# sieste/greb-climate-model

Measured on AMD Instinct MI355X. Metric: simulated-years/sec at 96x48 grid (ensemble aggregate); diffusion HBM GB/s vs roofline, higher is better.
Workload: dtype f32; 1 GPU; 96x48 GREB ensemble, 512 members/GPU x 1 GPU, CO2 sweep 280-1120 ppm, 32 scenario years after 1 flux-correction year, dt=12h, dt_crcl=0.5h; members_per_gpu=512, arithmetic=fast, gather=none (1 GPU)

## Files before the change

greb_climate_model_amd/csrc/greb_member.hip:

```cpp
#include <cstdlib>

#include "greb_kernels.h"
#include "greb_pair.h"
#include "greb_physics_step.h"
#include "greb_stencil.h"

namespace greb {

constexpr int NX = 96, NY = 48, NQ = 24, NP = 4608;
constexpr int kThreads = 512;
constexpr int RS = 2 * NX + 16;
constexpr int XB = (NY + 2) * RS;
constexpr int kOffX = RS;
constexpr int kOffW = 2 * XB + RS;
constexpr int kOffWX = 3 * XB;
constexpr int kOffWY = kOffWX + NP;
constexpr int kOffRowK = kOffWY + NP;
constexpr int kRowKCsDif = 7;
constexpr int kLdsFloats = kOffRowK + NY * kRowKWords;
constexpr size_t kLdsBytes = (size_t)kLdsFloats * sizeof(float);

bool member_layout_supported(const RowTables& t, int nx, int ny) {
  if (nx != NX || ny != NY) return false;
  for (int k = 0; k < NY; ++k) {
    const bool sub = (k <= 9 || k >= 38);
    if ((t.subcycled[k] != 0) != sub) return false;
    const bool chain = (k == 0 || k == NY - 1);
    if ((t.dif_time2[k] > 1 || t.adv_time2[k] > 1) != chain) return false;
  }
  if (t.dif_time2[0] != t.dif_time2[NY - 1] || t.adv_time2[0] != t.adv_time2[NY - 1]) return false;
  return true;
}

__device__ __forceinline__ f4 comp(const q8& q, int tr) {
  return tr == 0 ? f4{{q.v[0].x, q.v[1].x, q.v[2].x, q.v[3].x}} : f4{{q.v[0].y, q.v[1].y, q.v[2].y, q.v[3].y}};
}
__device__ __forceinline__ q8 zip(const f4& a, const f4& b) {
  q8 r;
#pragma unroll
  for (int i = 0; i < 4; ++i) r.v[i] = v2{a.v[i], b.v[i]};
  return r;
}

struct TaskAddr { int c, l, r, kq; };

__device__ __forceinline__ q8 ld8p(const lfloat* p) {
  const vfloat4 a = *(const __attribute__((address_space(3))) vfloat4*)p;
  const vfloat4 b = *(const __attribute__((address_space(3))) vfloat4*)(p + kHalfRow);
  q8 r;
  r.v[0] = v2{a.x, a.y}; r.v[1] = v2{a.z, a.w}; r.v[2] = v2{b.x, b.y}; r.v[3] = v2{b.z, b.w};
  return r;
}

template <bool SUB>
__device__ __forceinline__ q8 fast_row(const q8& LT, const q8& CT, const q8& RT, const q8& Tm2, const q8& Tm1, const q8& Tp1,
                                       const q8& Tp2, const q8& LW, const q8& CW, const q8& RW, const q8& Wm2, const q8& Wm1,
                                       const q8& Wp1, const q8& Wp2, const f4& xq, const f4& yq, const WindSigns& ws,
                                       bool last_quad, float cs_dif, float dif_ccy, bool calm_q) {
  v2 T[12], w[12];
#pragma unroll
  for (int j = 0; j < 4; ++j) {
    T[j] = LT.v[j]; T[4 + j] = CT.v[j]; T[8 + j] = RT.v[j];
    w[j] = LW.v[j]; w[4 + j] = CW.v[j]; w[8 + j] = RW.v[j];
  }
  return substep_pair<SUB>(T, w, Tm2, Tm1, Tp1, Tp2, Wm2, Wm1, Wp1, Wp2, xq.v, ws.x, yq.v, ws.y, cs_dif, dif_ccy, last_quad, calm_q);
}

__device__ __forceinline__ void st8p(lfloat* o, const q8& xn) {
  vfloat4 a, b;
  a.x = xn.v[0].x; a.y = xn.v[0].y; a.z = xn.v[1].x; a.w = xn.v[1].y;
  b.x = xn.v[2].x; b.y = xn.v[2].y; b.z = xn.v[3].x; b.w = xn.v[3].y;
  *(__attribute__((address_space(3))) vfloat4*)o = a;
  *(__attribute__((address_space(3))) vfloat4*)(o + kHalfRow) = b;
}

__device__ __forceinline__ q8 strict_row(const q8& LT, const q8& CT, const q8& RT, const q8& Tm2, const q8& Tm1, const q8& Tp1,
                                         const q8& Tp2, const q8& LW, const q8& CW, const q8& RW, const q8& Wm2, const q8& Wm1,
                                         const q8& Wp1, const q8& Wp2, const f4& xq, const f4& yq, int k, int q,
                                         const RowK& rk, bool calm_q) {
#pragma clang fp contract(off)
  q8 xn;
  v2 T[12], w[12];
#pragma unroll
  for (int j = 0; j < 4; ++j) {
    T[j] = LT.v[j]; T[4 + j] = CT.v[j]; T[8 + j] = RT.v[j];
    w[j] = LW.v[j]; w[4 + j] = CW.v[j]; w[8 + j] = RW.v[j];
  }
  v2 dTx[4], dTy[4], dd[4], da[4];
  dif_lon_strict(T, w, rk.dif_cc, dTx);
  if (rk.sub) {
    v2 T1h[4] = {T[4], T[5], T[6], T[7]};
    clamp_add(T1h, dTx);
#pragma unroll
    for (int i = 0; i < 4; ++i) dTx[i] = T1h[i] - T[4 + i];
  }
  dif_lat_strict(CT, Tm1, Tp1, Wm1, Wp1, rk.dif_ccy, k, NY, dTy);
#pragma unroll
  for (int i = 0; i < 4; ++i) dd[i] = CW.v[i] * (dTx[i] + dTy[i]);
  if (!rk.sub) {
    adv_lon_full_strict(T, w, xq.v, rk.adv_cc, dTx);
  } else {
    v2 T1h[4] = {T[4], T[5], T[6], T[7]};
    adv_lon_sub_strict(T, w, xq.v, rk.adv_cc, q == NQ - 1, dTx);
    clamp_add(T1h, dTx);
#pragma unroll
    for (int i = 0; i < 4; ++i) dTx[i] = T1h[i] - T[4 + i];
  }
  adv_lat_strict(CT, Tm2, Tm1, Tp1, Tp2, Wm2, Wm1, Wp1, Wp2, yq.v, rk.adv_ccy, k, NY, dTy);
#pragma unroll
  for (int i = 0; i < 4; ++i) {
    da[i] = dTx[i] + dTy[i];
    const v2 xd = T[4 + i] + dd[i];
    v2 x = xd + da[i];
    if (calm_q) x.y = xd.y;
    xn.v[i] = x;
  }
  return xn;
}

template <bool STRICT, bool SUB>
__device__ __forceinline__ q8 one_row(const q8& LT, const q8& CT, const q8& RT, const q8& Tm2, const q8& Tm1, const q8& Tp1,
                                      const q8& Tp2, const q8& LW, const q8& CW, const q8& RW, const q8& Wm2, const q8& Wm1,
                                      const q8& Wp1, const q8& Wp2, const f4& xq, const f4& yq, const WindSigns& ws, int k, int q,
                                      const RowK& rk, bool calm_q) {
  if (STRICT) return strict_row(LT, CT, RT, Tm2, Tm1, Tp1, Tp2, LW, CW, RW, Wm2, Wm1, Wp1, Wp2, xq, yq, k, q, rk, calm_q);
  return fast_row<SUB>(LT, CT, RT, Tm2, Tm1, Tp1, Tp2, LW, CW, RW, Wm2, Wm1, Wp1, Wp2, xq, yq, ws, q == NQ - 1, rk.dif_cc,
                       rk.dif_ccy, calm_q);
}

template <bool STRICT>
__device__ __forceinline__ RowK task_consts(const lfloat* lds, int k, float ccy_dif) {
  if (STRICT) return row_consts((const lfloat*)(lds + kOffRowK), k);
  RowK rk{};
  rk.dif_cc = lds[kOffRowK + k * kRowKWords + kRowKCsDif];
  rk.dif_ccy = ccy_dif;
  return rk;
}

template <bool STRICT, bool SUB>
__device__ __forceinline__ void row_task(lfloat* lds, int cur, const TaskAddr& ta, const WindSigns* ws, float ccy_dif,
                                         bool calm_q = false) {
  const int k = ta.kq & 255, q = ta.kq >> 8;
  const lfloat* Xc = lds + kOffX + cur * XB;
  const lfloat* Wc = lds + kOffW;
  const RowK rk = task_consts<STRICT>(lds, k, ccy_dif);
  const f4 xq = ld4(lds + kOffWX + k * NX + 4 * q), yq = ld4(lds + kOffWY + k * NX + 4 * q);
  const lfloat* xb = Xc + ta.c - 2 * RS;
  const lfloat* wb = Wc + ta.c - 2 * RS;
  const q8 Tm2 = ld8p(xb), Tm1 = ld8p(xb + RS), CT = ld8p(xb + 2 * RS), Tp1 = ld8p(xb + 3 * RS), Tp2 = ld8p(xb + 4 * RS);
  const q8 Wm2 = ld8p(wb), Wm1 = ld8p(wb + RS), CW = ld8p(wb + 2 * RS), Wp1 = ld8p(wb + 3 * RS), Wp2 = ld8p(wb + 4 * RS);
  const q8 LT = ld8p(Xc + ta.l), RT = ld8p(Xc + ta.r), LW = ld8p(Wc + ta.l), RW = ld8p(Wc + ta.r);
  const q8 xn = one_row<STRICT, SUB>(LT, CT, RT, Tm2, Tm1, Tp1, Tp2, LW, CW, RW, Wm2, Wm1, Wp1, Wp2, xq, yq, ws[0], k, q, rk,
                                     calm_q);
  st8p(lds + kOffX + (cur ^ 1) * XB + ta.c, xn);
}

template <bool STRICT, bool SUB>
__device__ __forceinline__ void row_task2(lfloat* lds, int cur, const TaskAddr& ta, const WindSigns* ws, float ccy_dif,
                                          bool calm_q = false) {
  const int k = ta.kq & 255, q = ta.kq >> 8;
  const lfloat* Xc = lds + kOffX + cur * XB;
  const lfloat* Wc = lds + kOffW;
  const lfloat* xb = Xc + ta.c - 2 * RS;
  const lfloat* wb = Wc + ta.c - 2 * RS;
  const q8 T0 = ld8p(xb), T1 = ld8p(xb + RS), T2 = ld8p(xb + 2 * RS), T3 = ld8p(xb + 3 * RS), T4 = ld8p(xb + 4 * RS);
  const q8 W0 = ld8p(wb), W1 = ld8p(wb + RS), W2 = ld8p(wb + 2 * RS), W3 = ld8p(wb + 3 * RS), W4 = ld8p(wb + 4 * RS);
  lfloat* out = lds + kOffX + (cur ^ 1) * XB + ta.c;
  {
    const q8 LT = ld8p(Xc + ta.l), RT = ld8p(Xc + ta.r), LW = ld8p(Wc + ta.l), RW = ld8p(Wc + ta.r);
    const f4 xq = ld4(lds + kOffWX + k * NX + 4 * q), yq = ld4(lds + kOffWY + k * NX + 4 * q);
    const RowK rk = task_consts<STRICT>(lds, k, ccy_dif);
    st8p(out, one_row<STRICT, SUB>(LT, T2, RT, T0, T1, T3, T4, LW, W2, RW, W0, W1, W3, W4, xq, yq, ws[0], k, q, rk, calm_q));
  }
  __builtin_amdgcn_sched_barrier(0);
  {
    const q8 T5 = ld8p(xb + 5 * RS), W5 = ld8p(wb + 5 * RS);
    const q8 LT = ld8p(Xc + ta.l + RS), RT = ld8p(Xc + ta.r + RS), LW = ld8p(Wc + ta.l + RS), RW = ld8p(Wc + ta.r + RS);
    const f4 xq = ld4(lds + kOffWX + (k + 1) * NX + 4 * q), yq = ld4(lds + kOffWY + (k + 1) * NX + 4 * q);
    const RowK rk = task_consts<STRICT>(lds, k + 1, ccy_dif);
    st8p(out + RS,
         one_row<STRICT, SUB>(LT, T3, RT, T1, T2, T4, T5, LW, W3, RW, W1, W2, W4, W5, xq, yq, ws[1], k + 1, q, rk, calm_q));
  }
}

struct BulkTasks { TaskAddr t[3]; };
struct BulkSigns { WindSigns s[3][2]; };

enum { kNone = 0, kS1 = 1, kF1 = 2, kST = 3, kFT = 4 };
struct Pass { int kind, index; };
__host__ __device__ constexpr Pass deal_fast(int wave, int i) {
  constexpr Pass none{kNone, 0};
#if defined(GREB_TUNING) && defined(GREB_DEAL_FAST)
  constexpr Pass t[8][3] = {GREB_DEAL_FAST};
#else
  constexpr Pass t[8][3] = {
       {{kST, 0}, {kF1, 0}, none},      {{kST, 2}, {kF1, 1}, none},
       {{kFT, 1}, {kF1, 3}, none},      {{kFT, 2}, {kS1, 0}, none},
       {{kST, 1}, none, none},          {{kFT, 0}, none, none},
       {none, none, none},              {{kF1, 2}, {kF1, 4}, none}};
#endif
  return t[wave][i];
}
__host__ __device__ constexpr Pass deal_strict(int wave, int i) {
  constexpr Pass none{kNone, 0};
  constexpr Pass t[8][3] = {
       {{kST, 0}, {kFT, 0}, none},      {{kST, 2}, {kF1, 0}, {kF1, 1}},
       {none, none, none},              {none, none, none},
       {{kST, 1}, none, none},          {{kF1, 2}, {kF1, 3}, none},
       {{kFT, 1}, {kS1, 0}, none},      {{kFT, 2}, {kF1, 4}, none}};
  return t[wave][i];
}
template <bool STRICT>
__host__ __device__ constexpr Pass deal(int wave, int i) { return STRICT ? deal_strict(wave, i) : deal_fast(wave, i); }
#if defined(GREB_TUNING) && defined(GREB_POLAR_WAVE_FAST)
constexpr int kPolarWaveFast = GREB_POLAR_WAVE_FAST;
#else
constexpr int kPolarWaveFast = 6;
#endif
template <bool STRICT>
__host__ __device__ constexpr bool is_polar_wave(int wave) { return STRICT ? (wave == 2 || wave == 3) : wave == kPolarWaveFast; }

struct RowQuad { int k, q, valid; };
__host__ __device__ constexpr int task_rows(int kind) { return kind == kST || kind == kFT ? 2 : (kind == kS1 || kind == kF1 ? 1 : 0); }
__host__ __device__ constexpr RowQuad task_rowquad(int kind, int t) {
  int k = 1, q = 0, valid = 0;
  const int r = t / NQ;
  q = t % NQ;
  if (kind == kST) { valid = r < 8; k = r < 4 ? 1 + 2 * r : (r == 4 ? 41 : (r == 5 ? 39 : (r == 6 ? 45 : 43))); }
  else if (kind == kFT) { valid = r < 8; k = 10 + 2 * r; }
  else if (kind == kS1) { valid = r < 2; k = r == 0 ? 9 : 38; if (r == 1) q = (q + 4) % NQ; }
  else if (kind == kF1) { valid = r < 12; k = r < 6 ? 26 + 2 * r : 27 + 2 * (r - 6); }
  if (!valid) { k = 1; q = 0; }
  return RowQuad{k, q, valid};
}

__host__ __device__ constexpr int kind_passes(int kind) { return kind == kST || kind == kFT ? 3 : (kind == kS1 ? 1 : (kind == kF1 ? 5 : 0)); }
__host__ __device__ constexpr int pass_tasks(int kind, int index) {
  const int total = kind == kST || kind == kFT ? 8 * NQ : (kind == kS1 ? 2 * NQ : (kind == kF1 ? 12 * NQ : 0));
  const int left = total - 64 * index;
  return left >= 64 ? 64 : (left > 0 ? left : 0);
}

struct DealCover { int n[NY * NQ]; };
template <bool STRICT>
__host__ __device__ constexpr DealCover deal_cover() {
  DealCover c{};
  for (int w = 0; w < 8; ++w)
    for (int i = 0; i < 3; ++i) {
      const Pass p = deal<STRICT>(w, i);
      if (p.kind == kNone) continue;
      for (int lane = 0; lane < 64; ++lane) {
        const RowQuad rq = task_rowquad(p.kind, 64 * p.index + lane);
        for (int j = 0; j < (rq.valid ? task_rows(p.kind) : 0); ++j) ++c.n[(rq.k + j) * NQ + rq.q];
      }
    }
  return c;
}
template <bool STRICT>
__host__ __device__ constexpr bool deal_is_complete() {
  for (int w = 0; w < 8; ++w)
    for (int i = 0; i < 3; ++i) {
      const Pass p = deal<STRICT>(w, i);
      if (is_polar_wave<STRICT>(w) && p.kind != kNone) return false;
      if (p.kind != kNone && (p.index < 0 || p.index >= kind_passes(p.kind))) return false;
    }
  const DealCover c = deal_cover<STRICT>();
  for (int k = 0; k < NY; ++k)
    for (int q = 0; q < NQ; ++q) if (c.n[k * NQ + q] != (k >= 1 && k <= NY - 2 ? 1 : 0)) return false;
  return true;
}
static_assert(deal_is_complete<true>() && deal_is_complete<false>(),
              "a deal must compute every row-quad of rows 1 .. 46 exactly once and give the polar waves no bulk pass");

void member_deal_cover(bool strict, int* counts) {
  constexpr DealCover cs = deal_cover<true>(), cf = deal_cover<false>();
  for (int i = 0; i < NY * NQ; ++i) counts[i] = strict ? cs.n[i] : cf.n[i];
}

template <bool STRICT>
__device__ __forceinline__ BulkTasks make_tasks(int wave, int lane) {
  BulkTasks b;
#pragma unroll
  for (int i = 0; i < 3; ++i) {
    const RowQuad rq = task_rowquad(deal<STRICT>(wave, i).kind, deal<STRICT>(wave, i).index * 64 + lane);
    const int k = rq.k, q = rq.q, valid = rq.valid;
    TaskAddr a;
    a.c = k * RS + 4 * q;
    a.l = k * RS + 4 * (q == 0 ? NQ - 1 : q - 1);
    a.r = k * RS + 4 * (q == NQ - 1 ? 0 : q + 1);
    a.kq = valid ? (k | (q << 8)) : -1;
    asm volatile("" : "+v"(a.c), "+v"(a.l), "+v"(a.r), "+v"(a.kq));
    b.t[i] = a;
  }
  return b;
}

template <int WAVE>
__device__ __forceinline__ void make_signs(const lfloat* lds, const BulkTasks& tasks, BulkSigns& b) {
  static_for<3>([&](auto I) {
    constexpr int i = I, rows = task_rows(deal_fast(WAVE, i).kind);
    if constexpr (rows > 0) {
      const int kq = tasks.t[i].kq < 0 ? 1 : tasks.t[i].kq, k = kq & 255, q = kq >> 8;
#pragma unroll
      for (int j = 0; j < rows; ++j) {
        const f4 xq = ld4(lds + kOffWX + (k + j) * NX + 4 * q), yq = ld4(lds + kOffWY + (k + j) * NX + 4 * q);
#pragma unroll
        for (int e = 0; e < 4; ++e) {
          unsigned long long mx = __builtin_amdgcn_ballot_w64(xq.v[e] > 0.f), my = __builtin_amdgcn_ballot_w64(yq.v[e] > 0.f);
          asm volatile("" : "+s"(mx), "+s"(my));
          b.s[i][j].x[e] = mx; b.s[i][j].y[e] = my;
        }
      }
    }
  });
}

template <bool STRICT, int SLOT, int I>
__device__ __forceinline__ void bulk_task(lfloat* lds, int cur, const BulkTasks& tasks, const BulkSigns& signs, float ccy_dif,
                                          int dbg, bool calm_q) {
  constexpr int kind = deal<STRICT>(SLOT, I).kind, ntask = pass_tasks(kind, deal<STRICT>(SLOT, I).index);
  if constexpr (kind != kNone && ntask > 0) {
    if (ntask < 64 && tasks.t[I].kq < 0) return;
    if constexpr (kind == kS1) { if (!(dbg & 1)) row_task<STRICT, true>(lds, cur, tasks.t[I], signs.s[I], ccy_dif, calm_q); }
    else if constexpr (kind == kF1) { if (!(dbg & 2)) row_task<STRICT, false>(lds, cur, tasks.t[I], signs.s[I], ccy_dif, calm_q); }
    else if constexpr (kind == kST) { if (!(dbg & 1)) row_task2<STRICT, true>(lds, cur, tasks.t[I], signs.s[I], ccy_dif, calm_q); }
    else { if (!(dbg & 2)) row_task2<STRICT, false>(lds, cur, tasks.t[I], signs.s[I], ccy_dif, calm_q); }
  }
}
template <bool STRICT, int SLOT>
__device__ __forceinline__ void bulk_substep(lfloat* lds, int cur, const BulkTasks& tasks, const BulkSigns& signs, float ccy_dif,
                                             int dbg, bool calm_q = false) {
  bulk_task<STRICT, SLOT, 0>(lds, cur, tasks, signs, ccy_dif, dbg, calm_q);
  bulk_task<STRICT, SLOT, 1>(lds, cur, tasks, signs, ccy_dif, dbg, calm_q);
  bulk_task<STRICT, SLOT, 2>(lds, cur, tasks, signs, ccy_dif, dbg, calm_q);
}

__device__ __forceinline__ int pair_off(int l) { return (l & 1) * kHalfRow + (l >> 1) * 4; }
__device__ __forceinline__ void load_win10(const lfloat* row, int l, v2 t[10]) {
  const int lm2 = l >= 2 ? l - 2 : l + 46, lm1 = l >= 1 ? l - 1 : 47, lp1 = l <= 46 ? l + 1 : 0, lp2 = l <= 45 ? l + 2 : l - 46;
  const int idx[5] = {lm2, lm1, l, lp1, lp2};
#pragma unroll
  for (int i = 0; i < 5; ++i) {
    const vfloat4 a = *(const __attribute__((address_space(3))) vfloat4*)(row + pair_off(idx[i]));
    t[2 * i] = v2{a.x, a.y}; t[2 * i + 1] = v2{a.z, a.w};
  }
}
__device__ __forceinline__ void st_pair2(lfloat* p, v2 a, v2 b) {
  vfloat4 x; x.x = a.x; x.y = a.y; x.z = b.x; x.w = b.y;
  *(__attribute__((address_space(3))) vfloat4*)p = x;
}

__device__ __forceinline__ void chain_substep_strict(lfloat* lds, int cur, int pole, int l , bool calm_q = false) {
  if (l >= 48) return;
  const int k = pole ? NY - 1 : 0;
  const RowK rk = row_consts((const lfloat*)(lds + kOffRowK), k);
  const lfloat* Xc = lds + kOffX + cur * XB;
  const lfloat* Wc = lds + kOffW;
  v2 T0w[10], w[10];
  load_win10(Xc + k * RS, l, T0w);
  load_win10(Wc + k * RS, l, w);
  const float u0 = lds[kOffWX + k * NX + 2 * l], u1 = lds[kOffWX + k * NX + 2 * l + 1];
  const float v0 = lds[kOffWY + k * NX + 2 * l], v1 = lds[kOffWY + k * NX + 2 * l + 1];
  const int k1 = pole ? k - 1 : k + 1, k2 = pole ? k - 2 : k + 2;
  v2 T1[2], T2[2], W1[2], W2[2];
  {
    const vfloat4 a = *(const __attribute__((address_space(3))) vfloat4*)(Xc + k1 * RS + pair_off(l));
    const vfloat4 b = *(const __attribute__((address_space(3))) vfloat4*)(Xc + k2 * RS + pair_off(l));
    const vfloat4 c = *(const __attribute__((address_space(3))) vfloat4*)(Wc + k1 * RS + pair_off(l));
    const vfloat4 d = *(const __attribute__((address_space(3))) vfloat4*)(Wc + k2 * RS + pair_off(l));
    T1[0] = v2{a.x, a.y}; T1[1] = v2{a.z, a.w}; T2[0] = v2{b.x, b.y}; T2[1] = v2{b.z, b.w};
    W1[0] = v2{c.x, c.y}; W1[1] = v2{c.z, c.w}; W2[0] = v2{d.x, d.y}; W2[1] = v2{d.z, d.w};
  }
  const v2 own[2] = {T0w[4], T0w[5]};
  const bool bug_lane = (l == 46);
  const int am2 = 4 * (l >= 2 ? l - 2 : l + 46), am1 = 4 * (l >= 1 ? l - 1 : 47), ap1 = 4 * (l <= 46 ? l + 1 : 0),
            ap2 = 4 * (l <= 45 ? l + 2 : l - 46);
  auto from = [](int addr, v2 x) {
    return v2{__int_as_float(__builtin_amdgcn_ds_bpermute(addr, __float_as_int(x.x))),
              __int_as_float(__builtin_amdgcn_ds_bpermute(addr, __float_as_int(x.y)))};
  };
  const float uu[2] = {u0, u1};

  v2 Th[2][2];
#pragma unroll
  for (int which = 0; which < 2; ++which) {
    const int time2 = __builtin_amdgcn_readfirstlane(which ? rk.adv_time2 : rk.dif_time2);
    const float cc = which ? rk.adv_cc : rk.dif_cc;
    v2 T[10];
#pragma unroll
    for (int i = 0; i < 10; ++i) T[i] = T0w[i];
    v2 th[2] = {own[0], own[1]};
    for (int tt = 0; tt < time2; ++tt) {
      if (tt > 0) {
        T[1] = from(am2, th[1]); T[2] = from(am1, th[0]); T[3] = from(am1, th[1]);
        T[4] = th[0]; T[5] = th[1];
        T[6] = from(ap1, th[0]); T[7] = from(ap1, th[1]); T[8] = from(ap2, th[0]);
      }
#pragma unroll
      for (int pt = 0; pt < 2; ++pt) {
#pragma clang fp contract(off)
        const int c = 4 + pt;
        v2 dd;
        if (which) dd = adv_lon_sub_point_strict(T, w, uu[pt], cc, c, bug_lane && pt == 1);
        else dd = div20(cc * dif_S_strict(T, w, c));
        dd = clamp_e(dd, T[c]);
        th[pt] = T[c] + dd;
      }
    }
    Th[which][0] = th[0]; Th[which][1] = th[1];
  }

  v2 xn[2];
  const float vv[2] = {v0, v1};
#pragma unroll
  for (int pt = 0; pt < 2; ++pt) {
#pragma clang fp contract(off)
    const v2 t0 = own[pt], w0 = w[4 + pt], a1 = T1[pt], a2 = T2[pt], b1 = W1[pt], b2 = W2[pt];
    const float vm = split_m(vv[pt]), vp = split_p(vv[pt]);
    v2 dTy, aTy;
    if (pole == 0) {
      dTy = rk.dif_ccy * b1 * (-t0 + a1);
      aTy = div3(rk.adv_ccy * (vp * (b1 * (t0 - a1) + b2 * (t0 - a2))));
    } else {
      dTy = rk.dif_ccy * b1 * (a1 - t0);
      aTy = div3(rk.adv_ccy * (-vm * (b1 * (t0 - a1) + b2 * (t0 - a2))));
    }
    const v2 dd = w0 * ((Th[0][pt] - t0) + dTy);
    const v2 da = (Th[1][pt] - t0) + aTy;
    const v2 xd = t0 + dd;
    v2 x = xd + da;
    if (calm_q) x.y = xd.y;
    xn[pt] = x;
  }
  st_pair2(lds + kOffX + (cur ^ 1) * XB + k * RS + pair_off(l), xn[0], xn[1]);
}

struct QuadChain {
  ChainK kd, ka;
  float w0[6], W1[6], W2[6];
  float own[6];
  float cv[6];
  float ccy;
  int at[3];
  int row[3];
  int time2_dif, time2_adv;
  bool calm;
};

__device__ __forceinline__ void quad_chain_setup(const lfloat* lds, int cur, int lane, bool calm_q, QuadChain& c) {
  const int r = lane >> 4, j = lane & 15, pole = r >> 1, C = r & 1;
  const int k = pole ? NY - 1 : 0, k1 = pole ? k - 1 : k + 1, k2 = pole ? k - 2 : k + 2;
  const RowK rk = row_consts((const lfloat*)(lds + kOffRowK), k);
  c.time2_dif = rk.dif_time2; c.time2_adv = rk.adv_time2; c.ccy = rk.dif_ccy;
  c.calm = calm_q && C == 1;
  c.row[0] = k * RS; c.row[1] = k1 * RS; c.row[2] = k2 * RS;
#pragma unroll
  for (int t = 0; t < 3; ++t) c.at[t] = pair_off(3 * j + t) + C;
  const lfloat* Wc = lds + kOffW;
  float w[12];
  static_for<12>([&](auto I) {
    constexpr int i = I;
    int x = 6 * j - 3 + i;
    x = x < 0 ? x + NX : (x >= NX ? x - NX : x);
    w[i] = Wc[c.row[0] + pair_off(x >> 1) + (x & 1) * 2 + C];
  });
  const float third = rk.adv_ccy * (1.f / 3.f), csd = rk.dif_cc * 0.05f, csa = rk.adv_cc * 0.05f;
  float Kd[6][6], Ka[6][6];
  static_for<6>([&](auto I) {
    constexpr int i = I, p = 3 + i;
    const int o = c.at[i >> 1] + (i & 1) * 2;
    c.w0[i] = w[p];
    c.own[i] = lds[kOffX + cur * XB + c.row[0] + o];
    c.W1[i] = Wc[c.row[1] + o];
    c.W2[i] = Wc[c.row[2] + o];
    const float u = lds[kOffWX + k * NX + 6 * j + i], v = lds[kOffWY + k * NX + 6 * j + i];
    c.cv[i] = pole == 0 ? third * fminf(v, 0.f) : -third * fmaxf(v, 0.f);
    Kd[i][0] = -csd * w[p - 3]; Kd[i][1] = (-3.f * csd) * w[p - 2]; Kd[i][2] = (-6.f * csd) * w[p - 1];
    Kd[i][3] = (6.f * csd) * w[p + 1]; Kd[i][4] = (3.f * csd) * w[p + 2]; Kd[i][5] = csd * w[p + 3];
    const float um = csa * fmaxf(u, 0.f), up = csa * fminf(u, 0.f);
    Ka[i][0] = -um * w[p - 3]; Ka[i][1] = (-4.f * um) * w[p - 2]; Ka[i][2] = (-10.f * um) * w[p - 1];
    Ka[i][3] = (-10.f * up) * w[p + 1]; Ka[i][4] = (-4.f * up) * w[p + 2]; Ka[i][5] = -up * w[p + 3];
    if (i == 3 && j == 15) {
      Ka[i][4] = -up * w[p + 3]; Ka[i][5] = -up * w[p + 3];
    }
  });
  c.kd = chain_pack(Kd);
  c.ka = chain_pack(Ka);
}

__device__ __forceinline__ void quad_chain_substep(lfloat* lds, int cur, QuadChain& c) {
  const lfloat* Xc = lds + kOffX + cur * XB;
  float own[6], T1[6], T2[6];
#pragma unroll
  for (int i = 0; i < 6; ++i) {
    const int o = c.at[i >> 1] + (i & 1) * 2;
    own[i] = c.own[i];
    T1[i] = Xc[c.row[1] + o];
    T2[i] = Xc[c.row[2] + o];
  }
  float Td[6], Ta[6];
#pragma unroll
  for (int i = 0; i < 6; ++i) { Td[i] = own[i]; Ta[i] = own[i]; }
  chain_run6<true>(Td, c.kd, c.time2_dif);
  chain_run6<true>(Ta, c.ka, c.time2_adv);
  lfloat* out = lds + kOffX + (cur ^ 1) * XB + c.row[0];
#pragma unroll
  for (int i = 0; i < 6; ++i) {
    const float g1 = c.W1[i] * (T1[i] - own[i]);
    const float d2 = c.W2[i] * (own[i] - T2[i]);
    const float ddy = c.ccy * g1;
    const float day = c.cv[i] * (d2 - g1);
    const float dd = c.w0[i] * ((Td[i] - own[i]) + ddy);
    float da = (Ta[i] - own[i]) + day;
    if (c.calm) da = 0.f;
    c.own[i] = (own[i] + dd) + da;
    out[c.at[i >> 1] + (i & 1) * 2] = c.own[i];
  }
}

template <bool STRICT, bool REMAT = false>
__device__ __forceinline__ void stage_winds(lfloat* lds, const float* __restrict__ u, const float* __restrict__ v,
                                            const RowTables* __restrict__ tab) {
  int tid0 = threadIdx.x;
  if (REMAT) asm volatile("" : "+v"(tid0));
  constexpr int kIt = (NP / 4 + kThreads - 1) / kThreads;
  f4 uq[kIt], vq[kIt];
#pragma unroll
  for (int j = 0; j < kIt; ++j) {
    const int i = min(tid0 + j * kThreads, NP / 4 - 1);
    uq[j] = ld4(u + 4 * i); vq[j] = ld4(v + 4 * i);
  }
#pragma unroll
  for (int j = 0; j < kIt; ++j) {
    const int i = tid0 + j * kThreads;
    if (i < NP / 4) {
      const int k = i / NQ;
      if (!(STRICT || k == 0 || k == NY - 1)) {
        const RowK rk = row_consts((const lfloat*)(lds + kOffRowK), k);
        const float cu = rk.sub ? rk.adv_cc * 0.05f : rk.adv_cc * (1.f / 3.f);
        const float cv = rk.adv_ccy * (1.f / 3.f);
#pragma unroll
        for (int e = 0; e < 4; ++e) { uq[j].v[e] *= cu; vq[j].v[e] *= cv; }
        if (k == 1 || k == NY - 2) {
#pragma unroll
          for (int e = 0; e < 4; ++e) {
            const float y = vq[j].v[e];
            vq[j].v[e] = (k == 1 ? y > 0.f : y < 0.f) ? 3.f * y : y;
          }
        }
      }
      st4(lds + kOffWX + 4 * i, uq[j]); st4(lds + kOffWY + 4 * i, vq[j]);
    }
  }
  (void)tab;
}

template <bool STRICT>
struct Circ {
  __device__ __forceinline__ void init(lfloat* lds, const float* wz_air, const float* wz_vapor,
                                       const RowTables* __restrict__ tab) {
    for (int i = threadIdx.x; i < 6 * RS; i += kThreads) {
      const int g = i / RS, o = i % RS;
      lds[(g >> 1) * XB + (g & 1) * (NY + 1) * RS + o] = 0.f;
    }
    stage_row_consts(lds + kOffRowK, *tab, 0, NY);
    if (!STRICT)
      for (int k = threadIdx.x; k < NY; k += blockDim.x)
        lds[kOffRowK + k * kRowKWords + kRowKCsDif] = lds[kOffRowK + k * kRowKWords] * 0.05f;
    for (int i = threadIdx.x; i < NP / 4; i += kThreads)
      st8(lds + kOffW + (i / NQ) * RS, i % NQ, zip(ld4(wz_air + 4 * i), ld4(wz_vapor + 4 * i)));
  }

  template <int WAVE, bool NOT_CALM>
  __device__ __forceinline__ void role_loop(lfloat* lds, int cur, int nsub, int lane, int dbg, bool calm_runtime
#ifdef GREB_TUNING
                                            , bool stamp, unsigned long long& busy
#endif
  ) {
    const bool calm_q = NOT_CALM ? false : calm_runtime;
    constexpr bool kPolar = is_polar_wave<STRICT>(WAVE);
    BulkTasks tasks;
    BulkSigns signs;
    QuadChain quad;
    if constexpr (!kPolar) tasks = make_tasks<STRICT>(WAVE, lane);
    else if constexpr (!STRICT) quad_chain_setup(lds, cur, lane, calm_q, quad);
    if constexpr (!kPolar && !STRICT) make_signs<WAVE>(lds, tasks, signs);
    float ccy_dif = 0.f;
    if constexpr (!kPolar && !STRICT) ccy_dif = __int_as_float(__builtin_amdgcn_readfirstlane(__float_as_int(lds[kOffRowK + 2])));
#pragma unroll 1
    for (int tt = 0; tt < nsub; ++tt) {
#ifdef GREB_TUNING
      const unsigned long long t0 = stamp ? __builtin_amdgcn_s_memtime() : 0;
#endif
      if constexpr (kPolar && STRICT) { if (!(dbg & 4)) chain_substep_strict(lds, cur, WAVE - 2, lane, calm_q); }
      else if constexpr (kPolar) { if (!(dbg & 4)) quad_chain_substep(lds, cur, quad); }
      else bulk_substep<STRICT, WAVE>(lds, cur, tasks, signs, ccy_dif, dbg, calm_q);
#ifdef GREB_TUNING
      if (stamp) busy += __builtin_amdgcn_s_memtime() - t0;
#endif
      __syncthreads();
      cur ^= 1;
    }
  }
  __device__ __forceinline__ void substeps(lfloat* lds, int cur, int nsub, int dbg = 0, bool calm_q = false
#ifdef GREB_TUNING
                                           , bool stamp = false, unsigned long long* busy = nullptr
#endif
  ) {
    int lane = threadIdx.x & 63;
    asm volatile("" : "+v"(lane));
#ifdef GREB_TUNING
    unsigned long long b = 0;
#define GREB_ROLE(W) case W: if (!STRICT && !calm_q) role_loop<W, true>(lds, cur, nsub, lane, dbg, false, stamp, b); \
                             else role_loop<W, false>(lds, cur, nsub, lane, dbg, calm_q, stamp, b); break;
#else
#define GREB_ROLE(W) case W: if (!STRICT && !calm_q) role_loop<W, true>(lds, cur, nsub, lane, dbg, false); \
                             else role_loop<W, false>(lds, cur, nsub, lane, dbg, calm_q); break;
#endif
    switch (__builtin_amdgcn_readfirstlane(threadIdx.x >> 6)) {
      GREB_ROLE(0) GREB_ROLE(1) GREB_ROLE(2) GREB_ROLE(3) GREB_ROLE(4) GREB_ROLE(5) GREB_ROLE(6) GREB_ROLE(7)
    }
#undef GREB_ROLE
#ifdef GREB_TUNING
    if (busy) *busy += b;
#endif
  }
};

template <bool STRICT>
__global__ __launch_bounds__(kThreads) void circulation_g96_kernel(const float* __restrict__ Xin,
                                                                   const float* __restrict__ wz,
                                                                   const float* __restrict__ ug,
                                                                   const float* __restrict__ vg,
                                                                   float* __restrict__ dX,
                                                                   const RowTables* __restrict__ tab, int nsub,
                                                                   int dbg) {
  extern __shared__ __align__(16) float lds_raw[];
  lfloat* lds = (lfloat*)lds_raw;
  const size_t fo = (size_t)blockIdx.x * NP;
  Circ<STRICT> c;
  c.init(lds, wz + fo, wz + fo, tab);
  for (int i = threadIdx.x; i < NP / 4; i += kThreads) {
    const f4 x = ld4(Xin + fo + 4 * i);
    st8(lds + kOffX + (i / NQ) * RS, i % NQ, zip(x, x));
  }
  __syncthreads();
  stage_winds<STRICT>(lds, ug + fo, vg + fo, tab);
  __syncthreads();
  c.substeps(lds, 0, nsub, dbg);
  const int cur = nsub & 1;
  for (int i = threadIdx.x; i < NP / 4; i += kThreads) {
    const f4 a = comp(ld8(lds + kOffX + cur * XB + (i / NQ) * RS, i % NQ), 0), b = ld4(Xin + fo + 4 * i);
    st4(dX + fo + 4 * i, f4{{a.v[0] - b.v[0], a.v[1] - b.v[1], a.v[2] - b.v[2], a.v[3] - b.v[3]}});
  }
}

hipError_t launch_circulation_g96(const float* X, const float* wz, const float* u, const float* v, float* dX,
                                  const RowTables* tab_dev, int batch, int nsub, bool strict, hipStream_t s) {
  auto kern = strict ? circulation_g96_kernel<true> : circulation_g96_kernel<false>;
  hipError_t e = hipFuncSetAttribute(reinterpret_cast<const void*>(kern),
                                     hipFuncAttributeMaxDynamicSharedMemorySize, (int)kLdsBytes);
  if (e != hipSuccess) return e;
  hipLaunchKernelGGL(kern, dim3(batch), dim3(kThreads), kLdsBytes, s, X, wz, u, v, dX, tab_dev, nsub,
                     tuning_int("GREB_DEBUG_SKIP", 0));
  return hipGetLastError();
}

template <bool STRICT, unsigned V>
__global__ __launch_bounds__(kThreads) void member_kernel(MemberArgs a) {
  constexpr bool FLUX = V & kVFlux, EXP = V & kVExp, BUDGET = V & kVBudget, FORCE = V & kVForce, BOUND = V & kVBound;
  extern __shared__ __align__(16) float lds_raw[];
  lfloat* lds = (lfloat*)lds_raw;
  const int m = blockIdx.x, tid = threadIdx.x;
  float* state = a.state + (size_t)m * 5 * NP;
  float* acc = a.acc + (size_t)m * 6 * NP;
  float* corr = a.corr + (size_t)a.corr_index[m] * 3 * kNT * NP;
  const RowTables* tab = a.tabs + a.tab_index[m];

#ifdef GREB_TUNING
  for (int i = 0; i < (a.dbg >> 8) * (m & 7); ++i) __builtin_amdgcn_s_sleep(16);
#endif
  Circ<STRICT> circ;
  const int bset = member_bset<BOUND>(a, m);
  {
    const BoundPtr B = member_boundary<BOUND>(a, bset);
    circ.init(lds, BOUND ? (const float*)B->wz_air : a.wz_air, BOUND ? (const float*)B->wz_vapor : a.wz_vapor, tab);
  }
  for (int i = tid; i < NP / 4; i += kThreads)
    st8(lds + kOffX + (i / NQ) * RS, i % NQ, zip(ld4(state + NP + 4 * i), ld4(state + 3 * NP + 4 * i)));
  int cur = 0;
  const unsigned xsw = EXP ? member_switches(a, m) : 0u;
  const int nsub = (EXP && (xsw & kXNoCirc)) ? 0 : a.nsub;
  const float co2_flux = FLUX ? (a.co2_flux_m ? a.co2_flux_m[m] : a.co2_flux) : 0.f;
  __syncthreads();
#ifdef GREB_TUNING
  const bool stamp = a.stamps != nullptr;
  unsigned long long st_wind = 0, st_circ = 0, st_busy = 0, st_phys = 0;
  const unsigned long long st_c0 = stamp ? __builtin_amdgcn_s_memtime() : 0, st_r0 = stamp ? __builtin_amdgcn_s_memrealtime() : 0;
#define GREB_STAMP(var) const unsigned long long var = stamp ? __builtin_amdgcn_s_memtime() : 0
#else
#define GREB_STAMP(var)
#endif

#pragma unroll 1
  for (int s = 0; s < a.nsteps; ++s) {
    const long long it = a.it0 + s;
    const StepClock ck = step_clock<FLUX>(a, it, NP);
    const int ityr = ck.ityr, yr_rel = ck.yr_rel;
    const size_t off = ck.off;

    GREB_STAMP(t_a);
    {
      const BoundPtr B = member_boundary<BOUND>(a, bset);
      stage_winds<STRICT, EXP && !STRICT>(lds, (BOUND ? (const float*)B->uclim : a.uclim) + off,
                                          (BOUND ? (const float*)B->vclim : a.vclim) + off, tab);
    }
    __syncthreads();
    GREB_STAMP(t_b);

#ifdef GREB_TUNING
    circ.substeps(lds, cur, nsub, 0, EXP && (xsw & kXQDiffOnly), stamp, &st_busy);
#else
    circ.substeps(lds, cur, nsub, 0, EXP && (xsw & kXQDiffOnly));
#endif
    cur ^= nsub & 1;
    GREB_STAMP(t_c);

    const Phys P = a.phys[m];
    const float co2 = FLUX ? co2_flux : a.co2[(size_t)m * a.co2_stride + a.co2_year0 + yr_rel];
    const MemberForce mf = member_force<FORCE>(a, m, ck);
    const BoundPtr B = member_boundary<BOUND>(a, bset);
    constexpr int ROUTE = STRICT ? kRouteArrays : kRouteRecord;
    const float* rec = nullptr;
    if constexpr (!STRICT) rec = member_record(a, bset);
    lfloat* Xf = lds + kOffX + cur * XB;
    lfloat* red = lds + kOffX + (cur ^ 1) * XB;
    if constexpr (BUDGET) {
      const BudgetSink bs = budget_sink<true>(a, m, ck);
#pragma unroll 1
      for (int qd = tid; qd < NP / 4; qd += kThreads) {
        const q8 xpair = ld8(Xf + (qd / NQ) * RS, qd % NQ);
        const PhysIn in = physics_load<V, ROUTE>(a, qd, ck, state, acc, corr, xsw, mf, B, rec);
        (void)physics_compute<STRICT, V | kVBudget, ROUTE>(a, P, in, co2, comp(xpair, 0), comp(xpair, 1), xsw, bs, 4 * qd, mf);
      }
    }
#pragma unroll 1
    for (int qd = tid; qd < NP / 4; qd += kThreads) {
#ifdef GREB_TUNING
      if ((a.dbg & 4) && qd >= kThreads) break;
#endif
      const q8 xpair = ld8(Xf + (qd / NQ) * RS, qd % NQ);
      f4 oTa, oq, tsm;
      physics_quad<STRICT, V & ~kVBudget, ROUTE>(a, P, m, qd, ck, co2, state, acc, corr, comp(xpair, 0), comp(xpair, 1), oTa, oq, tsm, xsw, mf, B, rec);
      st8(Xf + (qd / NQ) * RS, qd % NQ, zip(oTa, oq));
      if (ityr == kNT) st4(red + 4 * qd, tsm);
    }
    if (ityr == kNT) {
      __syncthreads();
      if (STRICT) {
        if (tid == 0 && a.yearly) {
#pragma clang fp contract(off)
          float sum = 0.f;
          for (int i = 0; i < NP; ++i) sum += red[i];
          float* y = a.yearly + ((size_t)m * a.yearly_years + (a.yearly_year0 + yr_rel)) * 2;
          y[0] = sum / (float)NP - 273.15f;
          y[1] = red[(a.ipy - 1) * NX + (a.ipx - 1)] - 273.15f;
        }
      } else if (a.yearly) {
        int t0 = tid;
        if (EXP) asm volatile("" : "+v"(t0));
        float part = 0.f;
        for (int i = t0; i < NP; i += kThreads) part += red[i];
        part = wave_sum(part);
        const float point = red[(a.ipy - 1) * NX + (a.ipx - 1)];
        __syncthreads();
        if ((tid & 63) == 0) red[tid >> 6] = part;
        __syncthreads();
        if (tid == 0) {
          float sum = 0.f;
          for (int w = 0; w < kThreads / 64; ++w) sum += red[w];
          float* y = a.yearly + ((size_t)m * a.yearly_years + (a.yearly_year0 + yr_rel)) * 2;
          y[0] = sum / (float)NP - 273.15f;
          y[1] = point - 273.15f;
        }
      }
    }
    __syncthreads();
#ifdef GREB_TUNING
    if (stamp) {
      const unsigned long long t_d = __builtin_amdgcn_s_memtime();
      st_wind += t_b - t_a; st_circ += t_c - t_b; st_phys += t_d - t_c;
    }
#endif
  }
#ifdef GREB_TUNING
  if (stamp && (tid & 63) == 0) {
    unsigned long long* o = a.stamps + ((size_t)m * (kThreads / 64) + (tid >> 6)) * 8;
    o[0] = __builtin_amdgcn_s_memtime() - st_c0; o[1] = __builtin_amdgcn_s_memrealtime() - st_r0;
    o[2] = st_wind; o[3] = st_circ; o[4] = st_busy; o[5] = st_phys; o[6] = (unsigned long long)a.nsteps; o[7] = (unsigned long long)nsub;
  }
#endif
}

static_assert(kFrNx == NX && kFrNy == NY, "the forcing record is the fused kernel's grid");
__global__ __launch_bounds__(256) void pack_forcing_kernel(BoundarySet b, float* __restrict__ rec) {
  const unsigned i = blockIdx.x * 256u + threadIdx.x;
  if (i >= (unsigned)kNT * NP) return;
  const unsigned step = i / NP, p = i - step * NP, row = p / NX, lon = p - row * NX;
  const unsigned prev = step > 0 ? step - 1 : kNT - 1;
  const float zt = b.z_topo[p];
  if (step == 0) {
    float* o = rec + forcing_record_offset((int)row, 0, (int)lon);
    o[forcing_record_offset(0, kFrZtopo, 0)] = zt;
    o[forcing_record_offset(0, kFrGlacier, 0)] = b.glacier[p];
    o[forcing_record_offset(0, kFrZocean, 0)] = b.z_ocean[p];
    o[forcing_record_offset(0, kFrWzAir, 0)] = b.wz_air[p];
  }
  float* o = rec + kFrStaticFloats + (size_t)step * kFrStepFloats + forcing_record_offset((int)row, kFrStaticFields, (int)lon);
  o[forcing_record_offset(0, kFrTclim, 0)] = b.tclim[i];
  o[forcing_record_offset(0, kFrCld, 0)] = b.cldclim[i];
  o[forcing_record_offset(0, kFrMld, 0)] = b.mldclim[i];
  o[forcing_record_offset(0, kFrMldPrev, 0)] = b.mldclim[(size_t)prev * NP + p];
  o[forcing_record_offset(0, kFrSwet, 0)] = b.swetclim[i];
  o[forcing_record_offset(0, kFrWind, 0)] = wind_speed<false>(b.uclim[i], b.vclim[i], zt);
}

hipError_t launch_pack_forcing(const BoundarySet& b, float* rec, hipStream_t s) {
  hipLaunchKernelGGL(pack_forcing_kernel, dim3((kNT * NP + 255) / 256), dim3(256), 0, s, b, rec);
  return hipGetLastError();
}

template <bool STRICT, unsigned V>
struct MemberFamily { static auto kernel() { return &member_kernel<STRICT, V>; } };

hipError_t launch_member_kernel(const MemberArgs& a, int n_members, bool strict, hipStream_t s) {
  if (a.nx != NX || a.ny != NY) return hipErrorInvalidValue;
  if (!strict && !a.bsets) return hipErrorInvalidValue;
  unsigned v;
  if (hipError_t e = select_variant(a, &v); e != hipSuccess) return e;
  const auto kern = pick_variant<MemberFamily>(strict, v);
  if (!kern) return hipErrorInvalidValue;
  hipError_t e = hipFuncSetAttribute(reinterpret_cast<const void*>(kern),
                                     hipFuncAttributeMaxDynamicSharedMemorySize, (int)kLdsBytes);
  if (e != hipSuccess) return e;
  hipLaunchKernelGGL(kern, dim3(n_members), dim3(kThreads), kLdsBytes, s, a);
  return hipGetLastError();
}

}
```

Baseline: 6011 simulated-years/s.

## Stage next step's winds in the physics tail on the last six waves

In the non-strict path, the next step's wind fields are now loaded and scaled into LDS by the last six waves (threads 128..511) at the end of the physics loop, instead of by every thread at the start of each step behind a separate barrier. The first step's winds are staged once before the loop. This removes one block-wide barrier per step and lets the wind loads overlap with waves still finishing physics. The tail waves take on three quads per thread instead of roughly three on average, and tuning stamps are extended to time the tail.

```diff
diff --git a/greb_climate_model_amd/csrc/greb_member.hip b/greb_climate_model_amd/csrc/greb_member.hip
--- a/greb_climate_model_amd/csrc/greb_member.hip
+++ b/greb_climate_model_amd/csrc/greb_member.hip
@@ -9,6 +9,7 @@
 
 constexpr int NX = 96, NY = 48, NQ = 24, NP = 4608;
 constexpr int kThreads = 512;
+constexpr int kMemberStampWords = 16;
 constexpr int RS = 2 * NX + 16;
 constexpr int XB = (NY + 2) * RS;
 constexpr int kOffX = RS;
@@ -271,6 +272,25 @@
 }
 static_assert(deal_is_complete<true>() && deal_is_complete<false>(),
               "a deal must compute every row-quad of rows 1 .. 46 exactly once and give the polar waves no bulk pass");
+
+__host__ __device__ constexpr int wind_quads_per_thread(int nt) { return (NP / 4 + nt - 1) / nt; }
+__host__ __device__ constexpr int wind_quad(int t0, int j, int nt) { return t0 + j * nt; }
+constexpr int kTailFirst = NP / 4 - 2 * kThreads;
+constexpr int kTailThreads = kThreads - kTailFirst;
+__host__ __device__ constexpr bool wind_cover_is_exact(int nt, int first) {
+  int n[NP / 4] = {};
+  for (int tid = first; tid < first + nt; ++tid)
+    for (int j = 0; j < wind_quads_per_thread(nt); ++j) {
+      const int i = wind_quad(tid - first, j, nt);
+      if (i < 0 || i >= NP / 4) return false;
+      ++n[i];
+    }
+  for (int i = 0; i < NP / 4; ++i) if (n[i] != 1) return false;
+  return true;
+}
+static_assert(kTailFirst == 128 && kTailFirst % 64 == 0 && kTailFirst + kTailThreads == kThreads &&
+                  wind_quads_per_thread(kTailThreads) == 3 && wind_cover_is_exact(kTailThreads, kTailFirst),
+              "the tail stages whole waves, three quads per thread and array, every one of the 1 152 quads exactly once");
 
 void member_deal_cover(bool strict, int* counts) {
   constexpr DealCover cs = deal_cover<true>(), cf = deal_cover<false>();
@@ -518,22 +538,24 @@
   }
 }
 
-template <bool STRICT, bool REMAT = false>
+template <bool STRICT, bool REMAT = false, int NT = kThreads, int T0 = 0>
 __device__ __forceinline__ void stage_winds(lfloat* lds, const float* __restrict__ u, const float* __restrict__ v,
                                             const RowTables* __restrict__ tab) {
   int tid0 = threadIdx.x;
   if (REMAT) asm volatile("" : "+v"(tid0));
-  constexpr int kIt = (NP / 4 + kThreads - 1) / kThreads;
+  if (T0) tid0 -= T0;
+  constexpr int kIt = wind_quads_per_thread(NT);
+  constexpr bool kExact = NP / 4 % NT == 0;
   f4 uq[kIt], vq[kIt];
 #pragma unroll
   for (int j = 0; j < kIt; ++j) {
-    const int i = min(tid0 + j * kThreads, NP / 4 - 1);
+    const int i = kExact ? wind_quad(tid0, j, NT) : min(wind_quad(tid0, j, NT), NP / 4 - 1);
     uq[j] = ld4(u + 4 * i); vq[j] = ld4(v + 4 * i);
   }
 #pragma unroll
   for (int j = 0; j < kIt; ++j) {
-    const int i = tid0 + j * kThreads;
-    if (i < NP / 4) {
+    const int i = wind_quad(tid0, j, NT);
+    if (kExact || i < NP / 4) {
       const int k = i / NQ;
       if (!(STRICT || k == 0 || k == NY - 1)) {
         const RowK rk = row_consts((const lfloat*)(lds + kOffRowK), k);
@@ -574,10 +596,13 @@
   template <int WAVE, bool NOT_CALM>
   __device__ __forceinline__ void role_loop(lfloat* lds, int cur, int nsub, int lane, int dbg, bool calm_runtime
 #ifdef GREB_TUNING
-                                            , bool stamp, unsigned long long& busy
+                                            , bool stamp, unsigned long long& busy, unsigned long long& first
 #endif
   ) {
     const bool calm_q = NOT_CALM ? false : calm_runtime;
+#ifdef GREB_TUNING
+    const unsigned long long t_call = stamp ? __builtin_amdgcn_s_memtime() : 0;
+#endif
     constexpr bool kPolar = is_polar_wave<STRICT>(WAVE);
     BulkTasks tasks;
     BulkSigns signs;
@@ -599,20 +624,23 @@
       if (stamp) busy += __builtin_amdgcn_s_memtime() - t0;
 #endif
       __syncthreads();
+#ifdef GREB_TUNING
+      if (stamp && tt == 0) first += __builtin_amdgcn_s_memtime() - t_call;
+#endif
       cur ^= 1;
     }
   }
   __device__ __forceinline__ void substeps(lfloat* lds, int cur, int nsub, int dbg = 0, bool calm_q = false
 #ifdef GREB_TUNING
-                                           , bool stamp = false, unsigned long long* busy = nullptr
+                                           , bool stamp = false, unsigned long long* busy = nullptr, unsigned long long* first = nullptr
 #endif
   ) {
     int lane = threadIdx.x & 63;
     asm volatile("" : "+v"(lane));
 #ifdef GREB_TUNING
-    unsigned long long b = 0;
-#define GREB_ROLE(W) case W: if (!STRICT && !calm_q) role_loop<W, true>(lds, cur, nsub, lane, dbg, false, stamp, b); \
-                             else role_loop<W, false>(lds, cur, nsub, lane, dbg, calm_q, stamp, b); break;
+    unsigned long long b = 0, f = 0;
+#define GREB_ROLE(W) case W: if (!STRICT && !calm_q) role_loop<W, true>(lds, cur, nsub, lane, dbg, false, stamp, b, f); \
+                             else role_loop<W, false>(lds, cur, nsub, lane, dbg, calm_q, stamp, b, f); break;
 #else
 #define GREB_ROLE(W) case W: if (!STRICT && !calm_q) role_loop<W, true>(lds, cur, nsub, lane, dbg, false); \
                              else role_loop<W, false>(lds, cur, nsub, lane, dbg, calm_q); break;
@@ -623,6 +651,7 @@
 #undef GREB_ROLE
 #ifdef GREB_TUNING
     if (busy) *busy += b;
+    if (first) *first += f;
 #endif
   }
 };
@@ -695,12 +724,31 @@
   __syncthreads();
 #ifdef GREB_TUNING
   const bool stamp = a.stamps != nullptr;
-  unsigned long long st_wind = 0, st_circ = 0, st_busy = 0, st_phys = 0;
+  unsigned long long st_wind = 0, st_circ = 0, st_busy = 0, st_phys = 0, st_quads = 0, st_tail = 0, st_wait = 0, st_first = 0;
   const unsigned long long st_c0 = stamp ? __builtin_amdgcn_s_memtime() : 0, st_r0 = stamp ? __builtin_amdgcn_s_memrealtime() : 0;
 #define GREB_STAMP(var) const unsigned long long var = stamp ? __builtin_amdgcn_s_memtime() : 0
 #else
 #define GREB_STAMP(var)
 #endif
+
+#ifdef GREB_TUNING
+  const bool tail = !STRICT && !(a.dbg & 8);
+#else
+  constexpr bool tail = !STRICT;
+#endif
+  if constexpr (!STRICT) {
+    if (tail) {
+      GREB_STAMP(t_a);
+      const BoundPtr B = member_boundary<BOUND>(a, bset);
+      const size_t off = step_clock<FLUX>(a, a.it0, NP).off;
+      stage_winds<STRICT, EXP>(lds, (BOUND ? (const float*)B->uclim : a.uclim) + off,
+                               (BOUND ? (const float*)B->vclim : a.vclim) + off, tab);
+      __syncthreads();
+#ifdef GREB_TUNING
+      if (stamp) st_wind += __builtin_amdgcn_s_memtime() - t_a;
+#endif
+    }
+  }
 
 #pragma unroll 1
   for (int s = 0; s < a.nsteps; ++s) {
@@ -710,16 +758,16 @@
     const size_t off = ck.off;
 
     GREB_STAMP(t_a);
-    {
+    if (!tail) {
       const BoundPtr B = member_boundary<BOUND>(a, bset);
       stage_winds<STRICT, EXP && !STRICT>(lds, (BOUND ? (const float*)B->uclim : a.uclim) + off,
                                           (BOUND ? (const float*)B->vclim : a.vclim) + off, tab);
-    }
-    __syncthreads();
+      __syncthreads();
+    }
     GREB_STAMP(t_b);
 
 #ifdef GREB_TUNING
-    circ.substeps(lds, cur, nsub, 0, EXP && (xsw & kXQDiffOnly), stamp, &st_busy);
+    circ.substeps(lds, cur, nsub, 0, EXP && (xsw & kXQDiffOnly), stamp, &st_busy, &st_first);
 #else
     circ.substeps(lds, cur, nsub, 0, EXP && (xsw & kXQDiffOnly));
 #endif
@@ -755,6 +803,16 @@
       st8(Xf + (qd / NQ) * RS, qd % NQ, zip(oTa, oq));
       if (ityr == kNT) st4(red + 4 * qd, tsm);
     }
+    GREB_STAMP(t_left);
+    if constexpr (!STRICT) {
+      if (tail && s + 1 < a.nsteps && __builtin_amdgcn_readfirstlane(threadIdx.x >> 6) >= kTailFirst / 64) {
+        const BoundPtr Bn = member_boundary<BOUND>(a, bset);
+        const size_t offn = step_clock<FLUX>(a, it + 1, NP).off;
+        stage_winds<false, EXP, kTailThreads, kTailFirst>(lds, (BOUND ? (const float*)Bn->uclim : a.uclim) + offn,
+                                                          (BOUND ? (const float*)Bn->vclim : a.vclim) + offn, tab);
+      }
+    }
+    GREB_STAMP(t_staged);
     if (ityr == kNT) {
       __syncthreads();
       if (STRICT) {
@@ -785,19 +843,23 @@
         }
       }
     }
+    GREB_STAMP(t_arrive);
     __syncthreads();
 #ifdef GREB_TUNING
     if (stamp) {
       const unsigned long long t_d = __builtin_amdgcn_s_memtime();
       st_wind += t_b - t_a; st_circ += t_c - t_b; st_phys += t_d - t_c;
+      st_quads += t_left - t_c; st_tail += t_staged - t_left; st_wait += t_d - t_arrive;
     }
 #endif
   }
 #ifdef GREB_TUNING
   if (stamp && (tid & 63) == 0) {
-    unsigned long long* o = a.stamps + ((size_t)m * (kThreads / 64) + (tid >> 6)) * 8;
+    unsigned long long* o = a.stamps + ((size_t)m * (kThreads / 64) + (tid >> 6)) * kMemberStampWords;
     o[0] = __builtin_amdgcn_s_memtime() - st_c0; o[1] = __builtin_amdgcn_s_memrealtime() - st_r0;
     o[2] = st_wind; o[3] = st_circ; o[4] = st_busy; o[5] = st_phys; o[6] = (unsigned long long)a.nsteps; o[7] = (unsigned long long)nsub;
+    o[8] = st_quads; o[9] = st_tail; o[10] = st_wait; o[11] = st_first;
+    for (int i = 12; i < kMemberStampWords; ++i) o[i] = 0;
   }
 #endif
 }
```

Result: no change. 6047 simulated-years/s, median of 2 (+0.6%).
